# NorthStarUAS/ImageAnalysis

Measured on AMD Instinct MI355X. Metric: image_pairs_matched_per_sec, higher is better.
Workload: dtype u8 (int8 MFMA, int32 accumulate)

## Files before the change

imageanalysis_amd/csrc/match_knn2sym.hip:

```cpp
#include "iamx_common.h"
#include "sym_cand_rule.h"

namespace {

typedef int v4i __attribute__((ext_vector_type(4)));
typedef int v2i __attribute__((ext_vector_type(2)));
typedef int v16i __attribute__((ext_vector_type(16)));
typedef unsigned v2u __attribute__((ext_vector_type(2)));

#ifndef IAMX_DESC_OFFSET
#define IAMX_DESC_OFFSET 128
#endif
constexpr int D = IAMX_DESC_DIM;
constexpr int CHUNK = 128;
constexpr int BIG = 0x3F000000;

struct Pack3Args {
    const void *src;
    const int64_t *src_off;
    int64_t single_n;
    const int32_t *dst_off;
    int8_t *dst;
    int32_t *sn2, *sct, *sperm, *sinv;
    int32_t *n2, *nb, *pos;
// ... 208 lines not shown
#if defined(IAMX_T_NOPACK)
    return U1;
#else
    typedef unsigned short us2 __attribute__((ext_vector_type(2)));
    const us2 d = __builtin_amdgcn_cvt_pk_u16((unsigned)(U1 - L), (unsigned)(U2 - L));
    return (int)__builtin_bit_cast(unsigned, d);
#endif
}
__device__ __forceinline__ void unpack_row_bounds(v2i e, int &L, int &U1, int &U2)
{
    const int d1 = e.y & 0xFFFF, d2 = (int)((unsigned)e.y >> 16);
    L = e.x;
    U1 = d1 == 0xFFFF ? ROW_NO_BOUND : e.x + d1;
    U2 = d2 == 0xFFFF ? ROW_NO_BOUND : e.x + d2;
}

struct SymArgs {
    const int8_t *sdesc;
    const int32_t *sn2, *sct;
    const int32_t *img_off, *img_n;
    const int32_t *upairs;
    const int32_t *wg_off;
    const int64_t *col_off;
    const int64_t *rowp_off;
    int32_t *col;
    int32_t *rowp;
    int n_u, total_wg;
    uint8_t *colmask;
#if defined(IAMX_T_STAMPS)
    unsigned long long *stamps;
#endif
};

__device__ __forceinline__ int uniform32(int x) { return __builtin_amdgcn_readfirstlane(x); }
__device__ __forceinline__ int64_t uniform64(int64_t x)
{
    return (int64_t)(((uint64_t)(unsigned)__builtin_amdgcn_readfirstlane((int)(x >> 32)) << 32) |
                     (unsigned)__builtin_amdgcn_readfirstlane((int)x));
}

template <bool FUSED>
__device__ __forceinline__ void half_wave_min16(int (&r)[16], int lo, int &m0, int &m1)
{
    int u[4], w[2];
    if constexpr (FUSED) {
        asm("s_nop 1\n\t"
            "v_min_i32_dpp %0, %0, %0 row_ror:8 row_mask:0xf bank_mask:0x3\n\t"
            "v_min_i32_dpp %0, %8, %8 row_ror:8 row_mask:0xf bank_mask:0xc\n\t"
            "v_min_i32_dpp %1, %1, %1 row_ror:8 row_mask:0xf bank_mask:0x3\n\t"
            "v_min_i32_dpp %1, %9, %9 row_ror:8 row_mask:0xf bank_mask:0xc\n\t"
            "v_min_i32_dpp %2, %2, %2 row_ror:8 row_mask:0xf bank_mask:0x3\n\t"
            "v_min_i32_dpp %2, %10, %10 row_ror:8 row_mask:0xf bank_mask:0xc\n\t"
            "v_min_i32_dpp %3, %3, %3 row_ror:8 row_mask:0xf bank_mask:0x3\n\t"
            "v_min_i32_dpp %3, %11, %11 row_ror:8 row_mask:0xf bank_mask:0xc\n\t"
            "v_min_i32_dpp %4, %4, %4 row_ror:8 row_mask:0xf bank_mask:0x3\n\t"
            "v_min_i32_dpp %4, %12, %12 row_ror:8 row_mask:0xf bank_mask:0xc\n\t"
            "v_min_i32_dpp %5, %5, %5 row_ror:8 row_mask:0xf bank_mask:0x3\n\t"
            "v_min_i32_dpp %5, %13, %13 row_ror:8 row_mask:0xf bank_mask:0xc\n\t"
            "v_min_i32_dpp %6, %6, %6 row_ror:8 row_mask:0xf bank_mask:0x3\n\t"
            "v_min_i32_dpp %6, %14, %14 row_ror:8 row_mask:0xf bank_mask:0xc\n\t"
            "v_min_i32_dpp %7, %7, %7 row_ror:8 row_mask:0xf bank_mask:0x3\n\t"
            "v_min_i32_dpp %7, %15, %15 row_ror:8 row_mask:0xf bank_mask:0xc"
            : "+v"(r[0]), "+v"(r[2]), "+v"(r[4]), "+v"(r[6]), "+v"(r[8]), "+v"(r[10]), "+v"(r[12]), "+v"(r[14])
            : "v"(r[1]), "v"(r[3]), "v"(r[5]), "v"(r[7]), "v"(r[9]), "v"(r[11]), "v"(r[13]), "v"(r[15]));
        asm("s_nop 1\n\t"
            "v_min_i32_dpp %0, %0, %0 row_ror:12 row_mask:0xf bank_mask:0x5\n\t"
// ... 93 lines not shown
            w[k] = min(w[k], __builtin_amdgcn_update_dpp(0, w[k], 0x4E, 0xF, 0xF, true));
        }
        dst[0] = w[0];
        dst[16] = w[1];
    }
}

template <int P, bool PASS>
__device__ __forceinline__ void row_min16_block(int (&r)[16], int &after)
{
    static_assert(P >= 0 && P < 6, "six blocks");
    int keep = after;
    if constexpr (P < 4) {
        asm("s_nop 1\n\t"
            "v_min_i32_dpp %0, %0, %0 row_ror:8 row_mask:0xf bank_mask:0x3\n\t"
            "v_min_i32_dpp %0, %3, %3 row_ror:8 row_mask:0xf bank_mask:0xc\n\t"
            "v_min_i32_dpp %1, %1, %1 row_ror:8 row_mask:0xf bank_mask:0x3\n\t"
            "v_min_i32_dpp %1, %4, %4 row_ror:8 row_mask:0xf bank_mask:0xc"
            : "+v"(r[4 * P]), "+v"(r[4 * P + 2]), "+v"(keep)
            : "v"(r[4 * P + 1]), "v"(r[4 * P + 3]));
    } else {
        constexpr int Q = 8 * (P - 4);
        asm("s_nop 1\n\t"
            "v_min_i32_dpp %0, %0, %0 row_ror:12 row_mask:0xf bank_mask:0x5\n\t"
            "v_min_i32_dpp %0, %3, %3 row_ror:4 row_mask:0xf bank_mask:0xa\n\t"
            "v_min_i32_dpp %1, %1, %1 row_ror:12 row_mask:0xf bank_mask:0x5\n\t"
            "v_min_i32_dpp %1, %4, %4 row_ror:4 row_mask:0xf bank_mask:0xa"
            : "+v"(r[Q]), "+v"(r[Q + 4]), "+v"(keep)
            : "v"(r[Q + 2]), "v"(r[Q + 6]));
    }
    if constexpr (PASS) after = keep;
}

template <int BYTES>
__device__ __forceinline__ void stage_piece_held(const void *gsrc, unsigned lds_dst, int &after)
{
    static_assert(BYTES == 16 || BYTES == 4, "one dwordx4 or one dword a lane");
    unsigned m0_was;
    int keep = after;
    if constexpr (BYTES == 16)
        asm volatile("s_mov_b32 %0, m0\n\ts_mov_b32 m0, %3\n\ts_nop 0\n\tglobal_load_lds_dwordx4 %2, off\n\ts_mov_b32 m0, %0"
                     : "=&s"(m0_was), "+v"(keep) : "v"(gsrc), "s"(lds_dst) : "memory");
    else
        asm volatile("s_mov_b32 %0, m0\n\ts_mov_b32 m0, %3\n\ts_nop 0\n\tglobal_load_lds_dword %2, off\n\ts_mov_b32 m0, %0"
                     : "=&s"(m0_was), "+v"(keep) : "v"(gsrc), "s"(lds_dst) : "memory");
    after = keep;
}

#if defined(IAMX_T_STAMPS)
#define SWEEP_STAMP(t)                                                                     \
    do {                                                                                   \
        __builtin_amdgcn_sched_barrier(0);                                                 \
        asm volatile("s_memtime %0\n\ts_waitcnt lgkmcnt(0)" : "=s"(t) : : "memory");       \
        __builtin_amdgcn_sched_barrier(0);                                                 \
    } while (0)
#endif

constexpr int sweep_gap_valu(int nv, int tail, bool blocks, int g)
{
    const int last = tail < 6 ? 6 - tail : 0;
    const int rest = nv - last - (blocks ? 2 : 0), n = blocks ? 5 : 7;
    if (g == 7) return last;
    if (blocks && (g == 3 || g == 4)) return 1;
    const int i = blocks && g > 4 ? g - 2 : g;
    return rest / n + (i < rest % n ? 1 : 0);
}

constexpr int sweep_min_order(bool blocks, int p3, int i)
{
    const int head = blocks ? 6 : 8;
    if (i < head) return 16 + i;
    if (blocks && (i == p3 || i == p3 + 1)) return 16 + 6 + (i - p3);
    const int f = i - (blocks && i < p3 ? 6 : 8);
    return f < 8 ? 24 + f : f - 8;
}

template <int V> struct int_c { static constexpr int value = V; };
template <int FROM, int TO, typename F>
// ... 15 lines not shown
    constexpr int WGROWS = NW * QW * 32;
    constexpr int NT = NW * 64;
    constexpr int PIECES = CHUNK * D / 16 / NT;
    __shared__ __attribute__((aligned(16))) int8_t lds[2 * CHUNK * D + 2 * CHUNK * 4 + 3 * NW * CHUNK * 4 + 2 * NW * 4 + (2 * NW * CHUNK + NW * 256) * 4];
    int8_t *lds_tile = lds;
    int *lds_tb = reinterpret_cast<int *>(lds + 2 * CHUNK * D);
    int *lds_row = lds_tb + 2 * CHUNK;
    int *lds_cq = lds_row + 3 * NW * CHUNK;
    int *lds_dump = lds_cq + 2 * NW;
    const int tid = threadIdx.x, lane = tid & 63, wave = tid >> 6;
    const int c = lane & 31, g = lane >> 5;

    int vid;
    {
        const int total = A.total_wg, bid = blockIdx.x;
        const int xcd = bid & 7, k = bid >> 3, q = total >> 3, r = total & 7;
        vid = (xcd < r ? xcd * (q + 1) : r * (q + 1) + (xcd - r) * q) + k;
    }
    int lo = 0, hi = A.n_u;
    if constexpr (!ITEMS)
        while (hi - lo > 1) {
            const int mid = (lo + hi) >> 1;
            if (A.wg_off[mid] <= vid) lo = mid; else hi = mid;
        }
    int u = lo, u_end = 0, item_wgi = 0;
    if constexpr (ITEMS) {
        u = A.wg_off[3 * vid];
        u_end = u + A.wg_off[3 * vid + 1];
        item_wgi = A.wg_off[3 * vid + 2];
    }
    v4i bq[QW][4];
    int lo_lane;
    int bimg_held = -1;
    if constexpr (ITEMS) asm volatile("" : "+v"(u_end), "+v"(item_wgi), "+v"(bimg_held));
#if defined(IAMX_T_STAMPS)
    unsigned long long stamp_sum = 0, stamp_chunks = 0, stamp_cycles = 0, stamp_ticks = 0;
#endif
    int nx_b = 0, nx_a = 0, nx_boff = 0, nx_nb = 0, nx_aoff = 0, nx_na = 0;
    int64_t nx_rowp = 0;
    if constexpr (ITEMS) {
        nx_b = A.upairs[2 * u];
        nx_a = A.upairs[2 * u + 1];
        nx_boff = A.img_off[nx_b];
        nx_nb = A.img_n[nx_b];
        nx_aoff = A.img_off[nx_a];
        nx_na = A.img_n[nx_a];
        nx_rowp = A.rowp_off[u];
    }
    for (;;) {
        const int bimg = ITEMS ? uniform32(nx_b) : A.upairs[2 * u], aimg = ITEMS ? uniform32(nx_a) : A.upairs[2 * u + 1];
        const int boff = ITEMS ? uniform32(nx_boff) : A.img_off[bimg], nb = ITEMS ? uniform32(nx_nb) : A.img_n[bimg];
        const int aoff = ITEMS ? uniform32(nx_aoff) : A.img_off[aimg], na = ITEMS ? uniform32(nx_na) : A.img_n[aimg];
        const int capA = (na + CHUNK - 1) / CHUNK * CHUNK;
        const int nchunks = capA / CHUNK;
        const int wgi = ITEMS ? uniform32(item_wgi) : vid - A.wg_off[u];
        const int q0 = wgi * WGROWS + wave * (QW * 32);
        const bool wave_valid = q0 < nb;
        const int64_t rbase = (ITEMS ? uniform64(nx_rowp) : A.rowp_off[u]) + (int64_t)wgi * capA;
        if constexpr (ITEMS)
            if (uniform32(bimg_held) >= 0) __syncthreads();

        const int rc = (c & 16) | ((c & 3) << 2) | ((c >> 2) & 3);
        if (!ITEMS || bimg != uniform32(bimg_held)) {
            bimg_held = bimg;
#pragma unroll
            for (int qb = 0; qb < QW; ++qb) {
                int row = q0 + QW * rc + qb;
                row = row < nb ? row : nb - 1;
                const v4i *src = reinterpret_cast<const v4i *>(A.sdesc + (int64_t)(boff + row) * D);
#pragma unroll
                for (int s = 0; s < 4; ++s) {
                    bq[qb][s] = ~src[2 * s + g];
                    if constexpr (WPE == 1) asm volatile("" : "+a"(bq[qb][s]));
                }
            }
            lo_lane = 0;
            {
                int spread = 0;
                if (wave_valid) {
                    const int g_lo = rc & ~3, g_hi = rc | 3;
                    const int r_lo = q0 + QW * g_lo < nb ? q0 + QW * g_lo : nb - 1;
                    const int r_hi = q0 + QW * g_hi + QW - 1 < nb ? q0 + QW * g_hi + QW - 1 : nb - 1;
                    lo_lane = A.sn2[boff + r_lo] >> 1;
                    spread = (A.sn2[boff + r_hi] >> 1) - lo_lane;
                }
#pragma unroll
                for (int sh = 32; sh >= 1; sh >>= 1) spread = max(spread, __shfl_xor(spread, sh));
                if (lane == 0) lds_cq[wave] = spread;
            }
        }
        if (!wave_valid) {
#pragma unroll
            for (int k = 0; k < 3 * CHUNK / 64; ++k)
                lds_row[((k / (CHUNK / 64)) * NW + wave) * CHUNK + (k % (CHUNK / 64)) * 64 + lane] = BIG;
        }
        int m[QW][4];
#pragma unroll
        for (int qb = 0; qb < QW; ++qb)
#pragma unroll
            for (int k = 0; k < 4; ++k) m[qb][k] = BIG;

        const int8_t *tbase = A.sdesc + (int64_t)aoff * D;
        const int32_t *tci = A.sct + aoff;
        typedef __attribute__((address_space(3))) void *lds_ptr;
        auto stage_direct = [&](int ch, int buf) {
#pragma unroll
            for (int j = 0; j < PIECES; ++j) {
                const int e = j * NT + tid, row = e >> 3, slot = (e & 7) ^ ((row >> 1) & 7);
                const int8_t *gsrc = tbase + (int64_t)(ch * CHUNK + row) * D + slot * 16;
                int8_t *ldst = lds_tile + buf * (CHUNK * D) + (j * NT + wave * 64) * 16;
                __builtin_amdgcn_global_load_lds(gsrc, (lds_ptr)ldst, 16, 0, 0);
            }
            __builtin_amdgcn_global_load_lds(tci + ch * CHUNK + (tid & (CHUNK - 1)),
                                             (lds_ptr)(lds_tb + buf * CHUNK + (wave & (CHUNK / 64 - 1)) * 64), 4, 0, 0);
        };
        auto wait_direct = [&]() { __builtin_amdgcn_s_waitcnt(0x0F70); };
        constexpr int MROWS = CHUNK / MERGEW;
        static_assert(MROWS == 64 && NW % MERGEW == 0, "one merge row per lane");
        const int mrow = (wave % MERGEW) * MROWS + lane;
        const bool merger = wave < MERGEW;
        constexpr int RSRC_WORD3_DATA_FORMAT_32 = 4 << 15;
        constexpr int RANGE_DROP = 0x7FFFFFF0;
        const __amdgpu_buffer_rsrc_t rowp_rsrc =
            __builtin_amdgcn_make_buffer_rsrc(A.rowp + 2 * rbase, (short)0, capA * 8, RSRC_WORD3_DATA_FORMAT_32);
        int spread_w[NW];
        auto merge_rows = [&](int ch, int rbo, bool store) {
            int L = BIG, U1 = BIG, U2 = BIG;
#pragma unroll
            for (int w = 0; w < NW; ++w) {
                const int R = lds_row[rbo + w * CHUNK + mrow];
                const int lw = R, uw = R + spread_w[w];
                L = min(L, lw);
                U2 = min(max(U1, uw), U2);
                U1 = min(U1, uw);
            }
            __builtin_amdgcn_raw_buffer_store_b64(v2i{L, pack_row_bounds(L, U1, U2)}, rowp_rsrc,
                                                  store ? (ch * CHUNK + mrow) * 8 : RANGE_DROP, 0, 0);
        };

        constexpr int PP = QW / 2, NT4 = CHUNK / 32, NS = NT4 * PP;
        static_assert(NT4 % 2 == 0 && NT4 >= 2, "tile parity must carry across chunks");
        int *const row_dst = (lane & 3) == 0 && wave_valid
            ? lds_row + wave * CHUNK + 8 * ((lane >> 4) & 1) + 4 * g + 2 * ((lane >> 2) & 1) + ((lane >> 3) & 1)
            : lds_dump + wave * 256 + lane;
        v4i aop[2][4], tbop[2][4];
        v16i accs[2][2];
        int r[2][16], bu[4];
#pragma unroll
        for (int k = 0; k < 16; ++k) r[1][k] = BIG;
        auto load_op = [&](int buf, int tile, int k, v4i (&a)[4], v4i (&tbv)[4]) {
            if (k < 4) {
                tbv[k] = *reinterpret_cast<const v4i *>(lds_tb + buf * CHUNK + tile * 32 + 8 * k + 4 * g);
            } else {
                const int s = k - 4, rr = tile * 32 + c, swz = (rr >> 1) & 7;
                a[s] = *reinterpret_cast<const v4i *>(lds_tile + buf * (CHUNK * D) + rr * D + (((2 * s + g) ^ swz) * 16));
            }
        };
        auto pin_accs = [&](v16i &acc0, v16i &acc1) {
            if constexpr (WPE == 1) asm volatile("" : "+v"(acc0), "+v"(acc1));
        };
        auto issue = [&](int t, int qp, v16i &acc0, v16i &acc1, bool pin = true) {
#pragma unroll
            for (int reg = 0; reg < 16; ++reg) acc0[reg] = acc1[reg] = tbop[t & 1][reg >> 2][reg & 3];
#pragma unroll
            for (int s = 0; s < 4; ++s) {
                acc0 = __builtin_amdgcn_mfma_i32_32x32x32_i8(aop[t & 1][s], bq[qp][s], acc0, 0, 0, 0);
                acc1 = __builtin_amdgcn_mfma_i32_32x32x32_i8(aop[t & 1][s], bq[qp + 1][s], acc1, 0, 0, 0);
            }
            if (pin) pin_accs(acc0, acc1);
        };

        if constexpr (ITEMS) {
            const int un = u + 1 < u_end ? u + 1 : u;
            nx_b = A.upairs[2 * un];
            nx_a = A.upairs[2 * un + 1];
            nx_rowp = A.rowp_off[un];
        }
        stage_direct(0, 0);
        stage_direct(nchunks > 1 ? 1 : 0, 1);
        wait_direct();
        __syncthreads();
#pragma unroll
        for (int w = 0; w < NW; ++w) spread_w[w] = __builtin_amdgcn_readfirstlane(lds_cq[w]);
        if constexpr (ITEMS) {
            const int b = uniform32(nx_b), a = uniform32(nx_a);
            nx_boff = A.img_off[b];
            nx_nb = A.img_n[b];
            nx_aoff = A.img_off[a];
            nx_na = A.img_n[a];
        }
#pragma unroll
        for (int k = 0; k < 8; ++k) load_op(0, 0, k, aop[0], tbop[0]);
#pragma unroll
        for (int k = 0; k < 8 / PP; ++k) load_op(0, 1, k, aop[1], tbop[1]);
        issue(0, 0, accs[0][0], accs[0][1]);
        __builtin_amdgcn_sched_barrier(0);
        int rbo = 0, rbo_prev = 2 * NW * CHUNK;
        const int wave_u = uniform32(wave);
        typedef __attribute__((address_space(3))) const int8_t *lds_bytes;
        int opoff[4], tboff = 2 * CHUNK * D + 16 * g;
#pragma unroll
        for (int s = 0; s < 4; ++s) opoff[s] = c * D + (((2 * s + g) ^ ((c >> 1) & 7)) * 16);
        auto load_op_at = [&](int tile, int k, v4i (&a)[4], v4i (&tbv)[4]) {
            if (k < 4) tbv[k] = *reinterpret_cast<const __attribute__((address_space(3))) v4i *>((lds_bytes)lds + tboff + tile * 128 + 32 * k);
            else a[k - 4] = *reinterpret_cast<const __attribute__((address_space(3))) v4i *>((lds_bytes)lds + opoff[k - 4] + tile * (32 * D));
        };
        const unsigned stage_voff = (unsigned)((tid >> 3) * D + (((tid & 7) ^ ((tid >> 4) & 7)) * 16));
        const unsigned lds_tile_at = (unsigned)(uintptr_t)(lds_ptr)(lds_tile + wave_u * (64 * 16));
        const unsigned lds_tb_at = (unsigned)(uintptr_t)(lds_ptr)(lds_tb + (wave_u & (CHUNK / 64 - 1)) * 64);
        const unsigned ct_voff = (unsigned)((tid & (CHUNK - 1)) * 4);
#if defined(IAMX_T_STAMPS)
        const unsigned long long loop_c0 = __builtin_amdgcn_s_memtime(), loop_r0 = __builtin_amdgcn_s_memrealtime();
        __builtin_amdgcn_s_waitcnt(0xC07F);
#endif
        for (int ch = 0; ch < nchunks; ++ch) {
            const int buf = ch & 1;
            if constexpr (PP == 4) {
            constexpr int BAR = (NT4 - 1) * PP - 1;
            static_assert(NW == 4 && PIECES == 4 && BAR + 4 < NS && (NT / 8) % 16 == 0, "the gaps below are form 2's");
            const int chs = ch + 2 < nchunks ? ch + 2 : nchunks - 1;
            const int8_t *const sg_tile = tbase + (int64_t)chs * (CHUNK * D);
            const int8_t *const sg_ct = reinterpret_cast<const int8_t *>(tci + chs * CHUNK);
            int mR[NW], mL = BIG, mU1 = BIG, mU2 = BIG;
            static_for<0, NS>([&](auto st_c) {
                constexpr int st = decltype(st_c)::value;
                constexpr int t = st / PP, ph = st % PP, qp = 2 * ph, cur = st & 1;
                constexpr int nst = st + 1 < NS ? st + 1 : 0;
#if defined(IAMX_T_STAMPS)
                unsigned long long stamp_t0 = 0, stamp_t1 = 0;
                if constexpr (IAMX_T_STAMPS == st + 1 || (st == BAR && IAMX_T_STAMPS == 17)) SWEEP_STAMP(stamp_t0);
                if constexpr (st == 0 && IAMX_T_STAMPS == 19) {
                    SWEEP_STAMP(stamp_t0);
                    SWEEP_STAMP(stamp_t1);
                    stamp_sum += stamp_t1 - stamp_t0;
                }
#endif
                if constexpr (st == BAR) {
                    __builtin_amdgcn_s_waitcnt(0x0070);
#if defined(IAMX_T_STAMPS)
                    if constexpr (IAMX_T_STAMPS == 17) {
                        SWEEP_STAMP(stamp_t1);
                        stamp_sum += stamp_t1 - stamp_t0;
                    }
                    if constexpr (IAMX_T_STAMPS == 18) SWEEP_STAMP(stamp_t0);
#endif
                    __syncthreads();
#if defined(IAMX_T_STAMPS)
                    if constexpr (IAMX_T_STAMPS == 18) {
                        SWEEP_STAMP(stamp_t1);
                        stamp_sum += stamp_t1 - stamp_t0;
                    }
#endif
                }
                issue(nst / PP, 2 * (nst % PP), accs[cur ^ 1][0], accs[cur ^ 1][1], false);
                auto operand_reads = [&]() {
                    static_for<(st == BAR - 1 ? 1 : 0), (st == BAR - 2 ? 2 : 1)>([&](auto d_c) {
                        constexpr int sr = st + decltype(d_c)::value;
                        constexpr int T = (sr + 1) / PP + 1, i = (sr + 1) % PP;
#pragma unroll
                        for (int k = i * 8 / PP; k < (i + 1) * 8 / PP; ++k) load_op_at(T % NT4, k, aop[T & 1], tbop[T & 1]);
                    });
                };
                if constexpr (st == BAR) {
#pragma unroll
                    for (int s = 0; s < 4; ++s) opoff[s] ^= CHUNK * D;
                    tboff ^= CHUNK * 4;
                }
                constexpr int nv = (ph == 2 ? 36 : ph == 3 ? 40 : 32) + (st == BAR + 2 ? 11 : 0) + (st == BAR + 3 ? 5 : 0) +
                                   (st >= BAR && st <= BAR + PIECES ? 1 : 0) +
                                   (st == NS - 1 ? 2 : 0);
                constexpr int tail = (st == BAR - 1 ? 0 : st == BAR - 2 ? 4 : 2) + (ph == 3 ? 1 + 2 : 0) +
                                     (st == BAR + 1 ? 2 : 0) + (st == BAR + 3 ? 1 : 0);
                constexpr bool staging = st >= BAR && st <= BAR + PIECES;
                constexpr int STAGE_GAP = 1, STAGE_AT = 8 + 1;
                constexpr int blk_at = sweep_gap_valu(nv, tail, true, 0) + sweep_gap_valu(nv, tail, true, 1) +
                                       sweep_gap_valu(nv, tail, true, 2) - (staging ? 2 : 0);
                static_assert(ph == 3 || (blk_at >= 6 && blk_at < 31), "gaps 3 and 4 hold the last two minima of column chain 0");
                const v16i acc0 = accs[cur][0], acc1 = accs[cur][1];
                int (&rc_)[16] = r[t & 1];
                int (&rp)[16] = r[(t + 1) & 1];
                static_for<0, 32>([&](auto i_c) {
                    constexpr int i = decltype(i_c)::value, op = sweep_min_order(ph < 3, blk_at, i);
                    if constexpr (op < 16) {
                        rc_[op] = qp == 0 ? min(acc0[op], acc1[op]) : min(min(rc_[op], acc0[op]), acc1[op]);
                    } else {
                        constexpr int w = op - 16;
                        int &mm = m[qp + (w >> 3)][t & 3];
                        const v16i &acc = w < 8 ? acc0 : acc1;
                        mm = min(min(mm, acc[2 * (w & 7)]), acc[2 * (w & 7) + 1]);
                        if constexpr (ph < 3 && i == blk_at) row_min16_block<2 * ph, true>(rp, mm);
                        if constexpr (ph < 3 && i == blk_at + 1) row_min16_block<2 * ph + 1, true>(rp, mm);
                        if constexpr (staging && w == STAGE_AT) {
                            if constexpr (st < BAR + PIECES)
                                stage_piece_held<16>(sg_tile + (st - BAR) * ((NT / 8) * D) + stage_voff,
                                                     lds_tile_at + buf * (CHUNK * D) + (st - BAR) * NT * 16, mm);
                            else
                                stage_piece_held<4>(sg_ct + ct_voff, lds_tb_at + buf * (CHUNK * 4), mm);
                        }
                    }
                });
                pin_accs(accs[cur ^ 1][0], accs[cur ^ 1][1]);
                operand_reads();
                if constexpr (ph == 2) {
#pragma unroll
                    for (int k = 0; k < 4; ++k) bu[k] = rp[4 * k] + lo_lane;
                }
                if constexpr (ph == 3) {
                    int *const dst = row_dst + (t > 0 ? rbo : rbo_prev) + (t > 0 ? t - 1 : NT4 - 1) * 32;
                    row_min16_piece<3>(rp, bu, lo_lane, dst);
                }
                if constexpr (st == BAR + 1) {
#pragma unroll
                    for (int w = 0; w < NW; ++w) mR[w] = lds_row[rbo_prev + w * CHUNK + mrow];
                }
                if constexpr (st == BAR + 2) {
#pragma unroll
                    for (int w = 0; w < NW; ++w) {
                        const int uw = mR[w] + spread_w[w];
                        mL = min(mL, mR[w]);
                        mU2 = min(max(mU1, uw), mU2);
                        mU1 = min(mU1, uw);
                    }
                }
                if constexpr (st == BAR + 3)
                    __builtin_amdgcn_raw_buffer_store_b64(v2i{mL, pack_row_bounds(mL, mU1, mU2)}, rowp_rsrc,
                                                          merger && ch > 0 ? ((ch - 1) * CHUNK + mrow) * 8 : RANGE_DROP, 0, 0);
                static_for<0, 8>([&](auto g_c) {
                    constexpr int g = decltype(g_c)::value;
                    __builtin_amdgcn_sched_group_barrier(0x008, 1, 0);
                    __builtin_amdgcn_sched_group_barrier(0x002, sweep_gap_valu(nv, tail, ph < 3, g) + (g == 7 ? 3 : 0) -
                                                                    (staging && g == STAGE_GAP ? 1 : 0), 0);
                });
                __builtin_amdgcn_sched_barrier(0);
#if defined(IAMX_T_STAMPS)
                if constexpr (IAMX_T_STAMPS == st + 1) {
                    SWEEP_STAMP(stamp_t1);
                    stamp_sum += stamp_t1 - stamp_t0;
                }
#endif
            });
            } else {
#pragma unroll
            for (int st = 0; st < NS; ++st) {
                const int t = st / PP, qp = 2 * (st % PP), cur = st & 1;
                if (st == (NT4 - 1) * PP - 1) {
                    __builtin_amdgcn_s_waitcnt(0x0070);
                    __syncthreads();
                    stage_direct(ch + 2 < nchunks ? ch + 2 : nchunks - 1, buf);
                    merge_rows(ch - 1, rbo_prev, merger && ch > 0);
                }
                if (st + 1 < NS) issue((st + 1) / PP, 2 * ((st + 1) % PP), accs[cur ^ 1][0], accs[cur ^ 1][1]);
                else issue(0, 0, accs[cur ^ 1][0], accs[cur ^ 1][1]);
                {
                    const int T = (st + 1) / PP + 1, i = (st + 1) % PP;
#pragma unroll
                    for (int k = i * 8 / PP; k < (i + 1) * 8 / PP; ++k)
                        load_op(T < NT4 ? buf : buf ^ 1, T % NT4, k, aop[T & 1], tbop[T & 1]);
                }
                const v16i acc0 = accs[cur][0], acc1 = accs[cur][1];
// ... 8 lines not shown
                m[qp + 1][t & 3] = t1m;
                int (&rc_)[16] = r[t & 1];
                if (qp == 0) {
#pragma unroll
                    for (int reg = 0; reg < 16; ++reg) rc_[reg] = min(acc0[reg], acc1[reg]);
                } else {
#pragma unroll
                    for (int reg = 0; reg < 16; ++reg) rc_[reg] = min(min(rc_[reg], acc0[reg]), acc1[reg]);
                }
                {
                    int (&rp)[16] = r[(t + 1) & 1];
                    const int tp = t > 0 ? t - 1 : NT4 - 1;
                    int *dst = row_dst + (t > 0 ? rbo : rbo_prev) + tp * 32;
                    if constexpr (PP == 1) {
                        int m0, m1;
                        half_wave_min16<true>(rp, lo_lane, m0, m1);
                        dst[0] = m0;
                        dst[16] = m1;
                    } else {
                        if (0 * PP / 4 == st % PP) row_min16_piece<0>(rp, bu, lo_lane, dst);
                        if (1 * PP / 4 == st % PP) row_min16_piece<1>(rp, bu, lo_lane, dst);
                        if (2 * PP / 4 == st % PP) row_min16_piece<2>(rp, bu, lo_lane, dst);
                        if (3 * PP / 4 == st % PP) row_min16_piece<3>(rp, bu, lo_lane, dst);
                    }
                }
#pragma unroll
                for (int i = 0; i < 8; ++i) {
                    __builtin_amdgcn_sched_group_barrier(0x008, 1, 0);
                    __builtin_amdgcn_sched_group_barrier(0x002, PIPE, 0);
                }
                __builtin_amdgcn_sched_barrier(0);
            }
            }
            rbo_prev = rbo;
            rbo = rbo == 2 * NW * CHUNK ? 0 : rbo + NW * CHUNK;
        }
#if defined(IAMX_T_STAMPS)
        if constexpr (PP == 4) {
            unsigned long long loop_c1;
            SWEEP_STAMP(loop_c1);
            stamp_cycles += loop_c1 - loop_c0;
            stamp_ticks += __builtin_amdgcn_s_memrealtime() - loop_r0;
            stamp_chunks += (unsigned)nchunks;
            if (A.stamps && lane == 0) {
                unsigned long long *o = A.stamps + ((size_t)blockIdx.x * NW + wave) * 4;
                o[0] = stamp_sum;
                o[1] = stamp_chunks;
                o[2] = stamp_cycles;
                o[3] = stamp_ticks;
            }
        }
#endif
        int64_t col_v = 0;
        if constexpr (ITEMS) col_v = A.col_off[u];
        {
            int m0, m1;
            half_wave_min16<true>(r[(NT4 - 1) & 1], lo_lane, m0, m1);
            int *dst = row_dst + rbo_prev + (NT4 - 1) * 32;
            dst[0] = m0;
            dst[16] = m1;
        }
        wait_direct();
        __syncthreads();
        merge_rows(nchunks - 1, rbo_prev, merger);

        const int64_t col_u = ITEMS ? uniform64(col_v) : 0;
        if (wave_valid) {
            unsigned ownpack = 0;
            int v1s[QW], v2s[QW];
#pragma unroll
            for (int qb = 0; qb < QW; ++qb) {
                const int lo01 = min(m[qb][0], m[qb][1]), hi01 = max(m[qb][0], m[qb][1]);
                const int lo23 = min(m[qb][2], m[qb][3]), hi23 = max(m[qb][2], m[qb][3]);
                const int a1 = min(lo01, lo23), a2 = min(max(lo01, lo23), min(hi01, hi23));
                const int b1 = __shfl_xor(a1, 32), b2 = __shfl_xor(a2, 32);
                const int v1 = min(a1, b1), v2 = min(max(a1, b1), min(a2, b2));
                v1s[qb] = v1;
                v2s[qb] = v2;
#if !defined(IAMX_T_NOMASK)
                const unsigned own = (m[qb][0] <= v2 ? 1u : 0u) | (m[qb][1] <= v2 ? 2u : 0u) |
                                     (m[qb][2] <= v2 ? 4u : 0u) | (m[qb][3] <= v2 ? 8u : 0u);
                ownpack |= own << (4 * qb);
#endif
            }
            const unsigned othpack = A.colmask ? (unsigned)__shfl_xor((int)ownpack, 32) : 0u;
            const int row0 = q0 + QW * rc;
            if (g == 0) {
#pragma unroll
                for (int qb = 0; qb < QW; ++qb)
                    if (row0 + qb < nb)
                        *reinterpret_cast<v2i *>(A.col + 2 * ((ITEMS ? col_u : A.col_off[u]) + row0 + qb)) = v2i{v1s[qb], v2s[qb]};
                if (A.colmask) {
                    uint8_t *dst = A.colmask + (ITEMS ? col_u : A.col_off[u]) + row0;
                    if (QW == 8 && row0 + QW <= nb) {
                        auto spread = [](unsigned nib4) {
                            const unsigned x = (nib4 | (nib4 << 8)) & 0x00FF00FFu;
                            return (x | (x << 4)) & 0x0F0F0F0Fu;
                        };
                        const unsigned lo = spread(ownpack & 0xFFFFu) | (spread(othpack & 0xFFFFu) << 4);
                        const unsigned hi = spread(ownpack >> 16) | (spread(othpack >> 16) << 4);
                        *reinterpret_cast<v2u *>(dst) = v2u{lo, hi};
                    } else {
#pragma unroll
                        for (int qb = 0; qb < QW; ++qb)
                            if (row0 + qb < nb)
                                dst[qb] = (uint8_t)(((ownpack >> (4 * qb)) & 15u) | (((othpack >> (4 * qb)) & 15u) << 4));
                    }
                }
            }
        }
        if constexpr (!ITEMS) break;
        else if (++u == uniform32(u_end)) break;
    }
}

struct NarTask { int p, cls, item0, n; };
struct NarLayout {
    int64_t ctl, pair_base, mask, slot, items, res, tasks, total;
    int64_t item_cap, task_cap;
};
__host__ __device__ inline NarLayout narrow_layout(int64_t rows, int64_t n_pairs)
{
    NarLayout L;
    auto up = [](int64_t v) { return (v + 255) / 256 * 256; };
    L.item_cap = rows;
    L.task_cap = rows / 64 + 80 * n_pairs + 64;
    int64_t o = 0;
    L.ctl = o;        o += 256;
    L.pair_base = o;  o += up(n_pairs * 4);
    L.mask = o;       o += up(rows * 8);
    L.slot = o;       o += up(rows * 8);
    L.items = o;      o += up(L.item_cap * 8);
    L.res = o;        o += up(L.item_cap * 16);
    L.tasks = o;      o += up(L.task_cap * 16);
    L.total = o;
    return L;
}
constexpr int NAR_MIN_TRAIN = 1024;
constexpr int NAR_ITEMS = 256;

struct CandArgs {
    const int32_t *sn2, *sperm, *img_off, *img_n;
    const int32_t *pairs;
    const int32_t *osrc;
    const int32_t *wg_off;
// ... 1225 lines not shown
```

Measured before the change: 631,100.

## Delay the row-bounds merge by one chunk and stream staging addresses incrementally

Moves the per-chunk row-minimum merge (LDS read, spread addition, min chain, buffer store) out of the barrier-adjacent steps to early steps of the following chunk, using a third rotating row buffer and a final merge after the loop. Staging addresses become scalar registers advanced in place inside the global_load_lds asm, and pointer advances are spread across steps. This is meant to cut the extra VALU and scalar work that clusters around the barrier window in the MFMA sweep. In exchange it adds register pressure, a tail merge, and fragile hand-tuned scheduling-gap counts.

```diff
diff --git a/imageanalysis_amd/csrc/match_knn2sym.hip b/imageanalysis_amd/csrc/match_knn2sym.hip
--- a/imageanalysis_amd/csrc/match_knn2sym.hip
+++ b/imageanalysis_amd/csrc/match_knn2sym.hip
@@ -423,18 +423,22 @@
     if constexpr (PASS) after = keep;
 }
 
-template <int BYTES>
-__device__ __forceinline__ void stage_piece_held(const void *gsrc, unsigned lds_dst, int &after)
+template <int BYTES, int NEXT>
+__device__ __forceinline__ void stage_piece_held(const void *sbase, unsigned voff, unsigned &lds_at, unsigned flip, int follows, int &after)
 {
     static_assert(BYTES == 16 || BYTES == 4, "one dwordx4 or one dword a lane");
     unsigned m0_was;
     int keep = after;
-    if constexpr (BYTES == 16)
-        asm volatile("s_mov_b32 %0, m0\n\ts_mov_b32 m0, %3\n\ts_nop 0\n\tglobal_load_lds_dwordx4 %2, off\n\ts_mov_b32 m0, %0"
-                     : "=&s"(m0_was), "+v"(keep) : "v"(gsrc), "s"(lds_dst) : "memory");
+    if constexpr (BYTES == 16 && NEXT > 0)
+        asm volatile("s_mov_b32 %0, m0\n\ts_mov_b32 m0, %2\n\ts_add_u32 %2, %2, %5\n\tglobal_load_lds_dwordx4 %3, %4\n\ts_mov_b32 m0, %0"
+                     : "=&s"(m0_was), "+v"(keep), "+s"(lds_at) : "v"(voff), "s"(sbase), "n"(NEXT), "v"(follows) : "memory", "scc");
+    else if constexpr (BYTES == 16)
+        asm volatile("s_mov_b32 %0, m0\n\ts_mov_b32 m0, %2\n\ts_sub_u32 %2, %5, %2\n\tglobal_load_lds_dwordx4 %3, %4\n\ts_mov_b32 m0, %0"
+                     : "=&s"(m0_was), "+v"(keep), "+s"(lds_at) : "v"(voff), "s"(sbase), "s"(flip), "v"(follows) : "memory", "scc");
     else
-        asm volatile("s_mov_b32 %0, m0\n\ts_mov_b32 m0, %3\n\ts_nop 0\n\tglobal_load_lds_dword %2, off\n\ts_mov_b32 m0, %0"
-                     : "=&s"(m0_was), "+v"(keep) : "v"(gsrc), "s"(lds_dst) : "memory");
+        asm volatile("s_mov_b32 %0, m0\n\ts_mov_b32 m0, %2\n\ts_sub_u32 %2, %5, %2\n\tglobal_load_lds_dword %3, %4\n\ts_mov_b32 m0, %0"
+                     : "=&s"(m0_was), "+v"(keep), "+s"(lds_at) : "v"(voff), "s"(sbase), "s"(flip), "v"(follows) : "memory", "scc");
+    static_assert(BYTES == 16 || NEXT == 0, "the Ct words are one piece");
     after = keep;
 }
 
@@ -680,6 +684,7 @@
         issue(0, 0, accs[0][0], accs[0][1]);
         __builtin_amdgcn_sched_barrier(0);
         int rbo = 0, rbo_prev = 2 * NW * CHUNK;
+        [[maybe_unused]] int rbo_pp = NW * CHUNK;
         const int wave_u = uniform32(wave);
         typedef __attribute__((address_space(3))) const int8_t *lds_bytes;
         int opoff[4], tboff = 2 * CHUNK * D + 16 * g;
@@ -693,6 +698,19 @@
         const unsigned lds_tile_at = (unsigned)(uintptr_t)(lds_ptr)(lds_tile + wave_u * (64 * 16));
         const unsigned lds_tb_at = (unsigned)(uintptr_t)(lds_ptr)(lds_tb + (wave_u & (CHUNK / 64 - 1)) * 64);
         const unsigned ct_voff = (unsigned)((tid & (CHUNK - 1)) * 4);
+        [[maybe_unused]] const int8_t *sg_tile = tbase + (int64_t)(nchunks > 1 ? 1 : 0) * (CHUNK * D);
+        [[maybe_unused]] const int8_t *sg_ct = reinterpret_cast<const int8_t *>(tci + (nchunks > 1 ? 1 : 0) * CHUNK);
+        [[maybe_unused]] unsigned stage_at = lds_tile_at, stage_ct_at = lds_tb_at;
+        [[maybe_unused]] const unsigned stage_flip = 2 * lds_tile_at + CHUNK * D + (PIECES - 1) * NT * 16;
+        [[maybe_unused]] const unsigned stage_ct_flip = 2 * lds_tb_at + CHUNK * 4;
+        [[maybe_unused]] unsigned piece_voff[PIECES];
+#pragma unroll
+        for (int j = 0; j < PIECES; ++j) {
+            piece_voff[j] = stage_voff + j * ((NT / 8) * D);
+            if constexpr (PP == 4) asm volatile("" : "+v"(piece_voff[j]));
+        }
+        [[maybe_unused]] int merge_voff = merger ? (mrow - 2 * CHUNK) * 8 : RANGE_DROP;
+        [[maybe_unused]] const int merge_vinc = merger ? CHUNK * 8 : 0;
 #if defined(IAMX_T_STAMPS)
         const unsigned long long loop_c0 = __builtin_amdgcn_s_memtime(), loop_r0 = __builtin_amdgcn_s_memrealtime();
         __builtin_amdgcn_s_waitcnt(0xC07F);
@@ -702,10 +720,11 @@
             if constexpr (PP == 4) {
             constexpr int BAR = (NT4 - 1) * PP - 1;
             static_assert(NW == 4 && PIECES == 4 && BAR + 4 < NS && (NT / 8) % 16 == 0, "the gaps below are form 2's");
-            const int chs = ch + 2 < nchunks ? ch + 2 : nchunks - 1;
-            const int8_t *const sg_tile = tbase + (int64_t)chs * (CHUNK * D);
-            const int8_t *const sg_ct = reinterpret_cast<const int8_t *>(tci + chs * CHUNK);
-            int mR[NW], mL = BIG, mU1 = BIG, mU2 = BIG;
+            constexpr int MRD = 1, MC0 = 4, MC1 = 5, MC2 = 8, MST = 9;
+            static_assert(MST + 1 < BAR && PP == 4, "the delayed merge ends in front of the barrier step");
+            int mR[NW], mU[NW], mL = BIG, mU1 = BIG, mU2 = BIG;
+            constexpr int ADV_TILE = 1, ADV_CT = 5;
+            int stage_adv = 0;
             static_for<0, NS>([&](auto st_c) {
                 constexpr int st = decltype(st_c)::value;
                 constexpr int t = st / PP, ph = st % PP, qp = 2 * ph, cur = st & 1;
@@ -737,6 +756,12 @@
 #endif
                 }
                 issue(nst / PP, 2 * (nst % PP), accs[cur ^ 1][0], accs[cur ^ 1][1], false);
+                if constexpr (nst == 0) {
+                    v16i c16;
+#pragma unroll
+                    for (int reg = 0; reg < 16; ++reg) c16[reg] = tbop[0][reg >> 2][reg & 3];
+                    asm volatile("" : : "v"(c16));
+                }
                 auto operand_reads = [&]() {
                     static_for<(st == BAR - 1 ? 1 : 0), (st == BAR - 2 ? 2 : 1)>([&](auto d_c) {
                         constexpr int sr = st + decltype(d_c)::value;
@@ -750,17 +775,19 @@
                     for (int s = 0; s < 4; ++s) opoff[s] ^= CHUNK * D;
                     tboff ^= CHUNK * 4;
                 }
-                constexpr int nv = (ph == 2 ? 36 : ph == 3 ? 40 : 32) + (st == BAR + 2 ? 11 : 0) + (st == BAR + 3 ? 5 : 0) +
-                                   (st >= BAR && st <= BAR + PIECES ? 1 : 0) +
+                constexpr int nv = (ph == 2 ? 36 : ph == 3 ? 40 : 32) +
+                                   (st == MRD ? 1 : 0) + (st == MC0 || st == MC1 || st == MST ? 4 : 0) + (st == MC2 ? 5 : 0) +
+                                   (st == MST + 1 ? 1 : 0) +
                                    (st == NS - 1 ? 2 : 0);
                 constexpr int tail = (st == BAR - 1 ? 0 : st == BAR - 2 ? 4 : 2) + (ph == 3 ? 1 + 2 : 0) +
-                                     (st == BAR + 1 ? 2 : 0) + (st == BAR + 3 ? 1 : 0);
+                                     (st == MRD ? 2 : 0) + (st == MST ? 1 : 0);
                 constexpr bool staging = st >= BAR && st <= BAR + PIECES;
                 constexpr int STAGE_GAP = 1, STAGE_AT = 8 + 1;
                 constexpr int blk_at = sweep_gap_valu(nv, tail, true, 0) + sweep_gap_valu(nv, tail, true, 1) +
-                                       sweep_gap_valu(nv, tail, true, 2) - (staging ? 2 : 0);
+                                       sweep_gap_valu(nv, tail, true, 2) - (staging ? 1 : 0);
                 static_assert(ph == 3 || (blk_at >= 6 && blk_at < 31), "gaps 3 and 4 hold the last two minima of column chain 0");
-                const v16i acc0 = accs[cur][0], acc1 = accs[cur][1];
+                v16i acc0 = accs[cur][0];
+                const v16i acc1 = accs[cur][1];
                 int (&rc_)[16] = r[t & 1];
                 int (&rp)[16] = r[(t + 1) & 1];
                 static_for<0, 32>([&](auto i_c) {
@@ -775,11 +802,13 @@
                         if constexpr (ph < 3 && i == blk_at) row_min16_block<2 * ph, true>(rp, mm);
                         if constexpr (ph < 3 && i == blk_at + 1) row_min16_block<2 * ph + 1, true>(rp, mm);
                         if constexpr (staging && w == STAGE_AT) {
+                            int lead = acc0[0];
                             if constexpr (st < BAR + PIECES)
-                                stage_piece_held<16>(sg_tile + (st - BAR) * ((NT / 8) * D) + stage_voff,
-                                                     lds_tile_at + buf * (CHUNK * D) + (st - BAR) * NT * 16, mm);
+                                stage_piece_held<16, (st < BAR + PIECES - 1 ? NT * 16 : 0)>(sg_tile, piece_voff[st - BAR], stage_at,
+                                                                                             stage_flip, mm, lead);
                             else
-                                stage_piece_held<4>(sg_ct + ct_voff, lds_tb_at + buf * (CHUNK * 4), mm);
+                                stage_piece_held<4, 0>(sg_ct, ct_voff, stage_ct_at, stage_ct_flip, mm, lead);
+                            acc0[0] = lead;
                         }
                     }
                 });
@@ -793,22 +822,32 @@
                     int *const dst = row_dst + (t > 0 ? rbo : rbo_prev) + (t > 0 ? t - 1 : NT4 - 1) * 32;
                     row_min16_piece<3>(rp, bu, lo_lane, dst);
                 }
-                if constexpr (st == BAR + 1) {
-#pragma unroll
-                    for (int w = 0; w < NW; ++w) mR[w] = lds_row[rbo_prev + w * CHUNK + mrow];
-                }
-                if constexpr (st == BAR + 2) {
-#pragma unroll
-                    for (int w = 0; w < NW; ++w) {
-                        const int uw = mR[w] + spread_w[w];
+                if constexpr (st == ADV_TILE) {
+                    stage_adv = ch + 2 < nchunks ? CHUNK * D : 0;
+                    sg_tile += stage_adv;
+                }
+                if constexpr (st == ADV_CT) sg_ct += stage_adv / (D / 4);
+                if constexpr (st == MRD) {
+#pragma unroll
+                    for (int w = 0; w < NW; ++w) mR[w] = lds_row[rbo_pp + w * CHUNK + mrow];
+                }
+                if constexpr (st == MC0) {
+#pragma unroll
+                    for (int w = 0; w < NW; ++w) mU[w] = mR[w] + spread_w[w];
+                }
+                if constexpr (st == MC1 || st == MC2) {
+                    constexpr int w0 = st == MC1 ? 0 : NW / 2;
+#pragma unroll
+                    for (int w = w0; w < w0 + NW / 2; ++w) {
                         mL = min(mL, mR[w]);
-                        mU2 = min(max(mU1, uw), mU2);
-                        mU1 = min(mU1, uw);
+                        mU2 = min(max(mU1, mU[w]), mU2);
+                        mU1 = min(mU1, mU[w]);
                     }
                 }
-                if constexpr (st == BAR + 3)
+                if constexpr (st == MST)
                     __builtin_amdgcn_raw_buffer_store_b64(v2i{mL, pack_row_bounds(mL, mU1, mU2)}, rowp_rsrc,
-                                                          merger && ch > 0 ? ((ch - 1) * CHUNK + mrow) * 8 : RANGE_DROP, 0, 0);
+                                                          (int)min((unsigned)merge_voff, (unsigned)RANGE_DROP), 0, 0);
+                if constexpr (st == MST + 1) merge_voff += merge_vinc;
                 static_for<0, 8>([&](auto g_c) {
                     constexpr int g = decltype(g_c)::value;
                     __builtin_amdgcn_sched_group_barrier(0x008, 1, 0);
@@ -883,8 +922,15 @@
                 __builtin_amdgcn_sched_barrier(0);
             }
             }
-            rbo_prev = rbo;
-            rbo = rbo == 2 * NW * CHUNK ? 0 : rbo + NW * CHUNK;
+            if constexpr (PP == 4) {
+                const int rbo_next = rbo_pp;
+                rbo_pp = rbo_prev;
+                rbo_prev = rbo;
+                rbo = rbo_next;
+            } else {
+                rbo_prev = rbo;
+                rbo = rbo == 2 * NW * CHUNK ? 0 : rbo + NW * CHUNK;
+            }
         }
 #if defined(IAMX_T_STAMPS)
         if constexpr (PP == 4) {
@@ -904,6 +950,7 @@
 #endif
         int64_t col_v = 0;
         if constexpr (ITEMS) col_v = A.col_off[u];
+        if constexpr (PP == 4) merge_rows(nchunks - 2, rbo_pp, merger && nchunks > 1);
         {
             int m0, m1;
             half_wave_min16<true>(r[(NT4 - 1) & 1], lo_lane, m0, m1);
```

After: 631,200 (median of 2 runs). Within noise of the previous version (+0.0%).

## Prefetch item table per wave and stage next pair's chunks across item boundaries

Applied to the files above, without the earlier changes.

In the persistent-items kernel, per-item metadata (image pairs, offsets, counts, rowp/col offsets) is now loaded once for up to 64 items into lanes and read with readlane, instead of issuing dependent scalar global loads each item. The chunk staging pipeline now continues across item boundaries, prefetching the next pair's first chunks during the tail of the current one. Double-buffer parity is tracked so the initial stage/wait/barrier is skipped when the B image is unchanged, and cached spread values are reused. This removes per-item pipeline drain and load latency, at the cost of more complex parity bookkeeping, extra registers and barrier changes.

```diff
diff --git a/imageanalysis_amd/csrc/match_knn2sym.hip b/imageanalysis_amd/csrc/match_knn2sym.hip
--- a/imageanalysis_amd/csrc/match_knn2sym.hip
+++ b/imageanalysis_amd/csrc/match_knn2sym.hip
@@ -264,6 +264,12 @@
 #endif
 };
 
+__device__ __forceinline__ void lds_barrier()
+{
+    __builtin_amdgcn_fence(__ATOMIC_RELEASE, "workgroup", "local");
+    __builtin_amdgcn_s_barrier();
+    __builtin_amdgcn_fence(__ATOMIC_ACQUIRE, "workgroup", "local");
+}
 __device__ __forceinline__ int uniform32(int x) { return __builtin_amdgcn_readfirstlane(x); }
 __device__ __forceinline__ int64_t uniform64(int64_t x)
 {
@@ -516,36 +522,112 @@
     v4i bq[QW][4];
     int lo_lane;
     int bimg_held = -1;
-    if constexpr (ITEMS) asm volatile("" : "+v"(u_end), "+v"(item_wgi), "+v"(bimg_held));
+    int tab_b = 0, tab_a = 0, tab_boff = 0, tab_nb = 0, tab_aoff = 0, tab_na = 0;
+    int64_t tab_rowp = 0, tab_col = 0;
+    auto load_item_table = [&](int first, int end) {
+        const int uj = first + lane < end ? first + lane : end - 1;
+        tab_b = A.upairs[2 * uj];
+        tab_a = A.upairs[2 * uj + 1];
+        tab_rowp = A.rowp_off[uj];
+        tab_col = A.col_off[uj];
+        tab_boff = A.img_off[tab_b];
+        tab_nb = A.img_n[tab_b];
+        tab_aoff = A.img_off[tab_a];
+        tab_na = A.img_n[tab_a];
+        asm volatile("" : "+v"(tab_b), "+v"(tab_a), "+v"(tab_boff), "+v"(tab_nb), "+v"(tab_aoff), "+v"(tab_na),
+                          "+v"(tab_rowp), "+v"(tab_col));
+    };
+    auto lane32 = [](int x, int l) { return __builtin_amdgcn_readlane(x, l); };
+    auto lane64 = [](int64_t x, int l) {
+        return (int64_t)(((uint64_t)(unsigned)__builtin_amdgcn_readlane((int)(x >> 32), l) << 32) |
+                         (unsigned)__builtin_amdgcn_readlane((int)x, l));
+    };
+    int tab_lane = 0, par_held = 0, nx_rows = 0, nx_chunks = 0;
+    if constexpr (ITEMS) {
+        load_item_table(u, u_end);
+        asm volatile("" : "+v"(u_end), "+v"(item_wgi), "+v"(bimg_held), "+v"(tab_lane), "+v"(par_held));
+    }
 #if defined(IAMX_T_STAMPS)
     unsigned long long stamp_sum = 0, stamp_chunks = 0, stamp_cycles = 0, stamp_ticks = 0;
 #endif
-    int nx_b = 0, nx_a = 0, nx_boff = 0, nx_nb = 0, nx_aoff = 0, nx_na = 0;
-    int64_t nx_rowp = 0;
-    if constexpr (ITEMS) {
-        nx_b = A.upairs[2 * u];
-        nx_a = A.upairs[2 * u + 1];
-        nx_boff = A.img_off[nx_b];
-        nx_nb = A.img_n[nx_b];
-        nx_aoff = A.img_off[nx_a];
-        nx_na = A.img_n[nx_a];
-        nx_rowp = A.rowp_off[u];
-    }
+    int spread_held[NW] = {};
     for (;;) {
-        const int bimg = ITEMS ? uniform32(nx_b) : A.upairs[2 * u], aimg = ITEMS ? uniform32(nx_a) : A.upairs[2 * u + 1];
-        const int boff = ITEMS ? uniform32(nx_boff) : A.img_off[bimg], nb = ITEMS ? uniform32(nx_nb) : A.img_n[bimg];
-        const int aoff = ITEMS ? uniform32(nx_aoff) : A.img_off[aimg], na = ITEMS ? uniform32(nx_na) : A.img_n[aimg];
+        const int tl = ITEMS ? uniform32(tab_lane) : 0;
+        const int bimg = ITEMS ? lane32(tab_b, tl) : A.upairs[2 * u], aimg = ITEMS ? lane32(tab_a, tl) : A.upairs[2 * u + 1];
+        const int boff = ITEMS ? lane32(tab_boff, tl) : A.img_off[bimg], nb = ITEMS ? lane32(tab_nb, tl) : A.img_n[bimg];
+        const int aoff = ITEMS ? lane32(tab_aoff, tl) : A.img_off[aimg], na = ITEMS ? lane32(tab_na, tl) : A.img_n[aimg];
         const int capA = (na + CHUNK - 1) / CHUNK * CHUNK;
         const int nchunks = capA / CHUNK;
         const int wgi = ITEMS ? uniform32(item_wgi) : vid - A.wg_off[u];
         const int q0 = wgi * WGROWS + wave * (QW * 32);
         const bool wave_valid = q0 < nb;
-        const int64_t rbase = (ITEMS ? uniform64(nx_rowp) : A.rowp_off[u]) + (int64_t)wgi * capA;
+        const int64_t rbase = (ITEMS ? lane64(tab_rowp, tl) : A.rowp_off[u]) + (int64_t)wgi * capA;
+        const bool fresh = !ITEMS || tl == 0;
+        const int par = ITEMS && !fresh ? uniform32(par_held) : 0;
+        int nxr = 0, nxn = 0;
+        if constexpr (ITEMS) {
+            if (u + 1 < uniform32(u_end) && tl + 1 < 64) {
+                nxr = lane32(tab_aoff, tl + 1) - aoff;
+                nxn = (lane32(tab_na, tl + 1) + CHUNK - 1) / CHUNK;
+            }
+            nx_rows = nxr;
+            nx_chunks = nxn;
+            par_held = par ^ (nchunks & 1);
+            asm volatile("" : "+v"(nx_rows), "+v"(nx_chunks), "+v"(par_held));
+        }
+        auto chunk_rows = [&](int w, int next_rows, int next_chunks) {
+            const int last = nchunks > 0 ? nchunks - 1 : 0, v = w - nchunks;
+            const int past = v < next_chunks ? next_rows + v * CHUNK : last * CHUNK;
+            return v < 0 ? w * CHUNK : past;
+        };
         if constexpr (ITEMS)
-            if (uniform32(bimg_held) >= 0) __syncthreads();
+            if (uniform32(bimg_held) >= 0) lds_barrier();
+
+        const int8_t *tbase = nullptr;
+        const int32_t *tci = nullptr;
+        auto stream_at = [&]() {
+            tbase = A.sdesc + (int64_t)aoff * D;
+            tci = A.sct + aoff;
+        };
+        if constexpr (ITEMS) stream_at();
+        typedef __attribute__((address_space(3))) void *lds_ptr;
+        auto stage_direct = [&](int ch, int buf) {
+#pragma unroll
+            for (int j = 0; j < PIECES; ++j) {
+                const int e = j * NT + tid, row = e >> 3, slot = (e & 7) ^ ((row >> 1) & 7);
+                const int8_t *gsrc = tbase + (int64_t)(ch * CHUNK + row) * D + slot * 16;
+                int8_t *ldst = lds_tile + buf * (CHUNK * D) + (j * NT + wave * 64) * 16;
+                __builtin_amdgcn_global_load_lds(gsrc, (lds_ptr)ldst, 16, 0, 0);
+            }
+            __builtin_amdgcn_global_load_lds(tci + ch * CHUNK + (tid & (CHUNK - 1)),
+                                             (lds_ptr)(lds_tb + buf * CHUNK + (wave & (CHUNK / 64 - 1)) * 64), 4, 0, 0);
+        };
+        auto wait_direct = [&]() { __builtin_amdgcn_s_waitcnt(0x0F70); };
+        if constexpr (ITEMS) {
+            auto stage_held = [&](int rows, int buf) {
+                int keep = 0;
+                const int wv = uniform32(wave);
+                const unsigned tile_at = (unsigned)(uintptr_t)(lds_ptr)(lds_tile + wv * (64 * 16)) + buf * (CHUNK * D);
+                const unsigned tb_at = (unsigned)(uintptr_t)(lds_ptr)(lds_tb + (wv & (CHUNK / 64 - 1)) * 64) + buf * (CHUNK * 4);
+                const unsigned voff = (unsigned)((tid >> 3) * D + (((tid & 7) ^ ((tid >> 4) & 7)) * 16));
+                const int8_t *src = tbase + (int64_t)rows * D;
+#pragma unroll
+                for (int j = 0; j < PIECES; ++j)
+                    stage_piece_held<16>(src + j * ((NT / 8) * D) + voff, tile_at + j * NT * 16, keep);
+                stage_piece_held<4>(reinterpret_cast<const int8_t *>(tci + rows) + (tid & (CHUNK - 1)) * 4, tb_at, keep);
+            };
+            if (fresh) {
+                stage_held(chunk_rows(0, nxr, nxn), 0);
+                stage_held(chunk_rows(1, nxr, nxn), 1);
+            } else if (nchunks == 1) {
+                stage_held(chunk_rows(1, nxr, nxn), par ^ 1);
+                wait_direct();
+            }
+        }
 
         const int rc = (c & 16) | ((c & 3) << 2) | ((c >> 2) & 3);
-        if (!ITEMS || bimg != uniform32(bimg_held)) {
+        const bool b_loads = !ITEMS || bimg != uniform32(bimg_held);
+        if (b_loads) {
             bimg_held = bimg;
 #pragma unroll
             for (int qb = 0; qb < QW; ++qb) {
@@ -555,8 +637,14 @@
 #pragma unroll
                 for (int s = 0; s < 4; ++s) {
                     bq[qb][s] = ~src[2 * s + g];
-                    if constexpr (WPE == 1) asm volatile("" : "+a"(bq[qb][s]));
-                }
+                    if constexpr (WPE == 1 && !ITEMS) asm volatile("" : "+a"(bq[qb][s]));
+                }
+            }
+            if constexpr (WPE == 1 && ITEMS) {
+#pragma unroll
+                for (int qb = 0; qb < QW; ++qb)
+#pragma unroll
+                    for (int s = 0; s < 4; ++s) asm volatile("" : "+a"(bq[qb][s]));
             }
             lo_lane = 0;
             {
@@ -584,21 +672,7 @@
 #pragma unroll
             for (int k = 0; k < 4; ++k) m[qb][k] = BIG;
 
-        const int8_t *tbase = A.sdesc + (int64_t)aoff * D;
-        const int32_t *tci = A.sct + aoff;
-        typedef __attribute__((address_space(3))) void *lds_ptr;
-        auto stage_direct = [&](int ch, int buf) {
-#pragma unroll
-            for (int j = 0; j < PIECES; ++j) {
-                const int e = j * NT + tid, row = e >> 3, slot = (e & 7) ^ ((row >> 1) & 7);
-                const int8_t *gsrc = tbase + (int64_t)(ch * CHUNK + row) * D + slot * 16;
-                int8_t *ldst = lds_tile + buf * (CHUNK * D) + (j * NT + wave * 64) * 16;
-                __builtin_amdgcn_global_load_lds(gsrc, (lds_ptr)ldst, 16, 0, 0);
-            }
-            __builtin_amdgcn_global_load_lds(tci + ch * CHUNK + (tid & (CHUNK - 1)),
-                                             (lds_ptr)(lds_tb + buf * CHUNK + (wave & (CHUNK / 64 - 1)) * 64), 4, 0, 0);
-        };
-        auto wait_direct = [&]() { __builtin_amdgcn_s_waitcnt(0x0F70); };
+        if constexpr (!ITEMS) stream_at();
         constexpr int MROWS = CHUNK / MERGEW;
         static_assert(MROWS == 64 && NW % MERGEW == 0, "one merge row per lane");
         const int mrow = (wave % MERGEW) * MROWS + lane;
@@ -608,6 +682,10 @@
         const __amdgpu_buffer_rsrc_t rowp_rsrc =
             __builtin_amdgcn_make_buffer_rsrc(A.rowp + 2 * rbase, (short)0, capA * 8, RSRC_WORD3_DATA_FORMAT_32);
         int spread_w[NW];
+        if constexpr (ITEMS) {
+#pragma unroll
+            for (int w = 0; w < NW; ++w) spread_w[w] = spread_held[w];
+        }
         auto merge_rows = [&](int ch, int rbo, bool store) {
             int L = BIG, U1 = BIG, U2 = BIG;
 #pragma unroll
@@ -654,44 +732,39 @@
             if (pin) pin_accs(acc0, acc1);
         };
 
-        if constexpr (ITEMS) {
-            const int un = u + 1 < u_end ? u + 1 : u;
-            nx_b = A.upairs[2 * un];
-            nx_a = A.upairs[2 * un + 1];
-            nx_rowp = A.rowp_off[un];
-        }
-        stage_direct(0, 0);
-        stage_direct(nchunks > 1 ? 1 : 0, 1);
-        wait_direct();
-        __syncthreads();
-#pragma unroll
-        for (int w = 0; w < NW; ++w) spread_w[w] = __builtin_amdgcn_readfirstlane(lds_cq[w]);
-        if constexpr (ITEMS) {
-            const int b = uniform32(nx_b), a = uniform32(nx_a);
-            nx_boff = A.img_off[b];
-            nx_nb = A.img_n[b];
-            nx_aoff = A.img_off[a];
-            nx_na = A.img_n[a];
-        }
-#pragma unroll
-        for (int k = 0; k < 8; ++k) load_op(0, 0, k, aop[0], tbop[0]);
-#pragma unroll
-        for (int k = 0; k < 8 / PP; ++k) load_op(0, 1, k, aop[1], tbop[1]);
+        if constexpr (!ITEMS) {
+            stage_direct(0, 0);
+            stage_direct(nchunks > 1 ? 1 : 0, 1);
+        }
+        if (fresh || b_loads) {
+            wait_direct();
+            __syncthreads();
+#pragma unroll
+            for (int w = 0; w < NW; ++w) spread_w[w] = __builtin_amdgcn_readfirstlane(lds_cq[w]);
+            if constexpr (ITEMS) {
+#pragma unroll
+                for (int w = 0; w < NW; ++w) spread_held[w] = spread_w[w];
+            }
+        }
+#pragma unroll
+        for (int k = 0; k < 8; ++k) load_op(par, 0, k, aop[0], tbop[0]);
+#pragma unroll
+        for (int k = 0; k < 8 / PP; ++k) load_op(par, 1, k, aop[1], tbop[1]);
         issue(0, 0, accs[0][0], accs[0][1]);
         __builtin_amdgcn_sched_barrier(0);
         int rbo = 0, rbo_prev = 2 * NW * CHUNK;
         const int wave_u = uniform32(wave);
         typedef __attribute__((address_space(3))) const int8_t *lds_bytes;
-        int opoff[4], tboff = 2 * CHUNK * D + 16 * g;
-#pragma unroll
-        for (int s = 0; s < 4; ++s) opoff[s] = c * D + (((2 * s + g) ^ ((c >> 1) & 7)) * 16);
+        int opoff[4], tboff = (2 * CHUNK * D + 16 * g) ^ (par * (CHUNK * 4));
+#pragma unroll
+        for (int s = 0; s < 4; ++s) opoff[s] = (c * D + (((2 * s + g) ^ ((c >> 1) & 7)) * 16)) ^ (par * (CHUNK * D));
         auto load_op_at = [&](int tile, int k, v4i (&a)[4], v4i (&tbv)[4]) {
             if (k < 4) tbv[k] = *reinterpret_cast<const __attribute__((address_space(3))) v4i *>((lds_bytes)lds + tboff + tile * 128 + 32 * k);
             else a[k - 4] = *reinterpret_cast<const __attribute__((address_space(3))) v4i *>((lds_bytes)lds + opoff[k - 4] + tile * (32 * D));
         };
         const unsigned stage_voff = (unsigned)((tid >> 3) * D + (((tid & 7) ^ ((tid >> 4) & 7)) * 16));
-        const unsigned lds_tile_at = (unsigned)(uintptr_t)(lds_ptr)(lds_tile + wave_u * (64 * 16));
-        const unsigned lds_tb_at = (unsigned)(uintptr_t)(lds_ptr)(lds_tb + (wave_u & (CHUNK / 64 - 1)) * 64);
+        const unsigned lds_tile_at = (unsigned)(uintptr_t)(lds_ptr)(lds_tile + wave_u * (64 * 16)) + par * (CHUNK * D);
+        const unsigned lds_tb_at = (unsigned)(uintptr_t)(lds_ptr)(lds_tb + (wave_u & (CHUNK / 64 - 1)) * 64) + par * (CHUNK * 4);
         const unsigned ct_voff = (unsigned)((tid & (CHUNK - 1)) * 4);
 #if defined(IAMX_T_STAMPS)
         const unsigned long long loop_c0 = __builtin_amdgcn_s_memtime(), loop_r0 = __builtin_amdgcn_s_memrealtime();
@@ -702,9 +775,19 @@
             if constexpr (PP == 4) {
             constexpr int BAR = (NT4 - 1) * PP - 1;
             static_assert(NW == 4 && PIECES == 4 && BAR + 4 < NS && (NT / 8) % 16 == 0, "the gaps below are form 2's");
-            const int chs = ch + 2 < nchunks ? ch + 2 : nchunks - 1;
-            const int8_t *const sg_tile = tbase + (int64_t)chs * (CHUNK * D);
-            const int8_t *const sg_ct = reinterpret_cast<const int8_t *>(tci + chs * CHUNK);
+            const int8_t *sg_tile = nullptr, *sg_ct = nullptr;
+            if constexpr (!ITEMS) {
+                const int chs = ch + 2 < nchunks ? ch + 2 : nchunks - 1;
+                sg_tile = tbase + (int64_t)chs * (CHUNK * D);
+                sg_ct = reinterpret_cast<const int8_t *>(tci + chs * CHUNK);
+            }
+            constexpr int SRC_AT = PP - 1;
+            auto stage_source = [&]() {
+                asm volatile("" : "+v"(nx_rows), "+v"(nx_chunks));
+                const int rows = chunk_rows(ch + 2, uniform32(nx_rows), uniform32(nx_chunks));
+                sg_tile = tbase + (int64_t)rows * D;
+                sg_ct = reinterpret_cast<const int8_t *>(tci + rows);
+            };
             int mR[NW], mL = BIG, mU1 = BIG, mU2 = BIG;
             static_for<0, NS>([&](auto st_c) {
                 constexpr int st = decltype(st_c)::value;
@@ -719,6 +802,7 @@
                     stamp_sum += stamp_t1 - stamp_t0;
                 }
 #endif
+                if constexpr (ITEMS && st == SRC_AT) stage_source();
                 if constexpr (st == BAR) {
                     __builtin_amdgcn_s_waitcnt(0x0070);
 #if defined(IAMX_T_STAMPS)
@@ -752,7 +836,8 @@
                 }
                 constexpr int nv = (ph == 2 ? 36 : ph == 3 ? 40 : 32) + (st == BAR + 2 ? 11 : 0) + (st == BAR + 3 ? 5 : 0) +
                                    (st >= BAR && st <= BAR + PIECES ? 1 : 0) +
-                                   (st == NS - 1 ? 2 : 0);
+                                   (st == NS - 1 ? 2 : 0) +
+                                   (ITEMS && st == SRC_AT ? 2 : 0);
                 constexpr int tail = (st == BAR - 1 ? 0 : st == BAR - 2 ? 4 : 2) + (ph == 3 ? 1 + 2 : 0) +
                                      (st == BAR + 1 ? 2 : 0) + (st == BAR + 3 ? 1 : 0);
                 constexpr bool staging = st >= BAR && st <= BAR + PIECES;
@@ -777,9 +862,11 @@
                         if constexpr (staging && w == STAGE_AT) {
                             if constexpr (st < BAR + PIECES)
                                 stage_piece_held<16>(sg_tile + (st - BAR) * ((NT / 8) * D) + stage_voff,
-                                                     lds_tile_at + buf * (CHUNK * D) + (st - BAR) * NT * 16, mm);
+                                                     (ITEMS ? lds_tile_at ^ (buf * (CHUNK * D)) : lds_tile_at + buf * (CHUNK * D)) +
+                                                         (st - BAR) * NT * 16, mm);
                             else
-                                stage_piece_held<4>(sg_ct + ct_voff, lds_tb_at + buf * (CHUNK * 4), mm);
+                                stage_piece_held<4>(sg_ct + ct_voff,
+                                                    ITEMS ? lds_tb_at ^ (buf * (CHUNK * 4)) : lds_tb_at + buf * (CHUNK * 4), mm);
                         }
                     }
                 });
@@ -902,8 +989,6 @@
             }
         }
 #endif
-        int64_t col_v = 0;
-        if constexpr (ITEMS) col_v = A.col_off[u];
         {
             int m0, m1;
             half_wave_min16<true>(r[(NT4 - 1) & 1], lo_lane, m0, m1);
@@ -915,7 +1000,7 @@
         __syncthreads();
         merge_rows(nchunks - 1, rbo_prev, merger);
 
-        const int64_t col_u = ITEMS ? uniform64(col_v) : 0;
+        const int64_t col_u = ITEMS ? lane64(tab_col, uniform32(tab_lane)) : 0;
         if (wave_valid) {
             unsigned ownpack = 0;
             int v1s[QW], v2s[QW];
@@ -961,7 +1046,16 @@
             }
         }
         if constexpr (!ITEMS) break;
-        else if (++u == uniform32(u_end)) break;
+        else {
+            if (++u == uniform32(u_end)) break;
+            int tn = uniform32(tab_lane) + 1;
+            if (tn == 64) {
+                load_item_table(u, uniform32(u_end));
+                tn = 0;
+            }
+            tab_lane = tn;
+            asm volatile("" : "+v"(tab_lane));
+        }
     }
 }
 
```

New measurement: 616,500 before, 618,700 after, median of 6. About the same (+0.4%).
